# jason-huang03/SPH_Project

Hardware: AMD Instinct MI355X
Metric: particle-updates/sec (higher is better)
Workload: dtype f32

## Files before the change

### include/sph_hip.h

```cpp
#ifndef SPH_HIP_H
#define SPH_HIP_H
#include <stddef.h>
#include <stdint.h>
#ifdef __cplusplus
extern "C" {
#endif

#define SPH_MAX_OBJECTS 20
#define SPH_MAT_FLUID 1
#define SPH_MAT_RIGID 2

typedef enum {
    SPH_OK = 0,
    SPH_ERR_INVALID = -1,
    SPH_ERR_CAPACITY = -2,
    SPH_ERR_HIP = -3,
    SPH_ERR_NO_DEVICE = -4,
    SPH_ERR_COMM = -5,
    SPH_ERR_UNSUPPORTED = -6
} SphStatus;

typedef enum { SPH_METHOD_WCSPH = 0, SPH_METHOD_DFSPH = 1, SPH_METHOD_PCISPH = 2, SPH_METHOD_IISPH = 3, SPH_METHOD_PBF = 4 } SphMethod;

typedef struct {
// ... 81 lines not shown
} SphPhase;

typedef struct {
    int64_t steps;
    int64_t pair_interactions;
    int32_t particle_num;
    int32_t fluid_particle_num;
    int32_t iter_divergence, iter_density, iter_pcisph, iter_cg;
    float   err_divergence, err_density, err_pcisph, err_cg;
    int64_t lds_fallback_blocks;
    double  total_time;
    int64_t pair_evaluations;
    int64_t hash_launches;
    int64_t prehashed_sorts;
    int64_t list_sorts;
    int32_t iter_iisph;
    float   err_iisph;
    int64_t pbf_recentred;
} SphStats;

typedef enum {
    SPH_K_HASH_COUNT = 0, SPH_K_SCAN = 1, SPH_K_SCATTER = 2, SPH_K_DENSITY = 3,
    SPH_K_NON_PRESSURE = 4, SPH_K_PRESSURE_INTEGRATE = 5, SPH_K_RIGID_VOLUME = 6,
    SPH_K_DFSPH_DENSITY_ALPHA = 7, SPH_K_DFSPH_RHO_ADV = 8, SPH_K_DFSPH_CORRECT = 9,
    SPH_K_REDUCE = 10, SPH_K_PCISPH_RHO_STAR = 11, SPH_K_PCISPH_PRESSURE_ACCEL = 12,
    SPH_K_CG_PREPARE = 13, SPH_K_CG_AP = 14, SPH_K_CG_VECTOR = 15, SPH_K_MISC = 16,
    SPH_K_HALO = 17, SPH_K_WCSPH_FORCES = 18,
    SPH_K_IISPH_PREPARE = 19, SPH_K_IISPH_DIJ_PJ = 20, SPH_K_IISPH_SUM_I = 21,
    SPH_K_PBF_DENSITY_LAMBDA = 22, SPH_K_PBF_FIX_POSITION = 23, SPH_K_PBF_UPDATE = 24,
    SPH_K_RIGID_CONTACT = 25, SPH_K_RIGID_INTEGRATE = 26, SPH_K_RIGID_CONTACT_SOLVE = 27, SPH_K_COUNT_
// ... 362 lines not shown
```

### sph_project_amd/_lib.py

```python
from __future__ import annotations

import ctypes as C
import os

import numpy as np

_HERE = os.path.dirname(os.path.abspath(__file__))
LIB_PATH = os.environ.get("SPH_HIP_LIB", os.path.join(_HERE, "libsph_hip.so"))

MAX_OBJECTS = 20
MAT_FLUID, MAT_RIGID = 1, 2
METHOD = {"wcsph": 0, "dfsph": 1, "pcisph": 2, "iisph": 3, "pbf": 4}

(F_POSITION, F_VELOCITY, F_ACCELERATION, F_DENSITY, F_PRESSURE, F_REST_VOLUME, F_MASS, F_MATERIAL,
 F_OBJECT_ID, F_IS_DYNAMIC, F_COLOR, F_PARTICLE_ID, F_GRID_ID, F_DFSPH_ALPHA, F_DFSPH_KAPPA,
 F_DFSPH_KAPPA_V, F_DENSITY_STAR, F_DENSITY_DERIV, F_PRESSURE_ACCEL, F_PREDICTED_VEL, F_PREDICTED_POS,
 F_CG_X, F_ORIG_POSITION, F_GHOST, F_DFSPH_KAPPA_NEXT, F_DFSPH_KAPPA_V_NEXT, F_DEBUG_CAPTURE,
 F_IISPH_DII, F_IISPH_AII, F_IISPH_DIJ_PJ, F_IISPH_SUM_I, F_PBF_OLD_POSITION, F_PBF_LAMBDA, F_RIGID_CONTACT_DN,
 F_RIGID_CONTACT_COUNT) = range(35)

_FIELD_SPEC = {
    F_POSITION: (np.float32, 3), F_VELOCITY: (np.float32, 3), F_ACCELERATION: (np.float32, 3),
    F_DENSITY: (np.float32, 1), F_PRESSURE: (np.float32, 1), F_REST_VOLUME: (np.float32, 1),
    F_MASS: (np.float32, 1), F_MATERIAL: (np.int32, 1), F_OBJECT_ID: (np.int32, 1),
# ... 34 lines not shown
        ("viscosity_b", C.c_double), ("density_0", C.c_double), ("surface_tension", C.c_double),
        ("dt", C.c_double), ("particle_max_num", C.c_int32), ("viscosity_implicit", C.c_int32),
        ("method", C.c_int32), ("fixed_iterations", C.c_int32), ("fast_math", C.c_int32),
        ("device", C.c_int32), ("force_global", C.c_int32), ("deterministic", C.c_int32),
    ]


class SphStats(C.Structure):
    _fields_ = [
        ("steps", C.c_int64), ("pair_interactions", C.c_int64), ("particle_num", C.c_int32),
        ("fluid_particle_num", C.c_int32), ("iter_divergence", C.c_int32), ("iter_density", C.c_int32),
        ("iter_pcisph", C.c_int32), ("iter_cg", C.c_int32), ("err_divergence", C.c_float),
        ("err_density", C.c_float), ("err_pcisph", C.c_float), ("err_cg", C.c_float),
        ("lds_fallback_blocks", C.c_int64), ("total_time", C.c_double), ("pair_evaluations", C.c_int64),
        ("hash_launches", C.c_int64), ("prehashed_sorts", C.c_int64), ("list_sorts", C.c_int64),
        ("iter_iisph", C.c_int32), ("err_iisph", C.c_float), ("pbf_recentred", C.c_int64),
    ]


class SphSurfaceParams(C.Structure):
    _fields_ = [
        ("radius", C.c_double), ("smoothing_length", C.c_double), ("cube_size", C.c_double), ("iso", C.c_double),
        ("normals", C.c_int32), ("fast_math", C.c_int32), ("device", C.c_int32), ("reserved", C.c_int32),
        ("memory_cap_bytes", C.c_int64),
    ]


class SphSurfaceStats(C.Structure):
    _fields_ = [
        ("particles", C.c_int64), ("active_bricks", C.c_int64), ("points_evaluated", C.c_int64), ("pair_tests", C.c_int64),
        ("vertices", C.c_int64), ("triangles", C.c_int64), ("bytes_allocated", C.c_int64), ("B", C.c_int32), ("reserved", C.c_int32),
# ... 555 lines not shown
```

### sph_project_amd/csrc/sph_api.hip

```cpp
#include "../../include/sph_hip.h"
#include "sph_common.hpp"
#include "sph_comm.hpp"

#include <math.h>
#include <stdarg.h>
#include <stdio.h>
#include <string.h>
#include <string>
#include <vector>
#include <stdlib.h>
#include <utility>
#include <array>
#include <algorithm>
#include "sph_voxel.hpp"
#include "sph_export.hpp"
#include "sph_devobj.hpp"

struct ProfSlot {
    bool on = false;
    int64_t launches = 0;
    double ms = 0.0;
    std::vector<std::pair<hipEvent_t, hipEvent_t>> pending;
};

// ... 737 lines not shown
    if (e == hipSuccess) e = hipMemcpyAsync(b, a, bytes, hipMemcpyDeviceToDevice, st);
    if (e == hipSuccess) e = hipEventRecord(e0, st);
    for (int k = 0; k < reps && e == hipSuccess; ++k) e = hipMemcpyAsync((k & 1) ? a : b, (k & 1) ? b : a, bytes, hipMemcpyDeviceToDevice, st);
    if (e == hipSuccess) e = hipEventRecord(e1, st);
    if (e == hipSuccess) e = hipStreamSynchronize(st);
    float ms = 0.0f;
    if (e == hipSuccess) e = hipEventElapsedTime(&ms, e0, e1);
    h->ev_pool.push_back(e0); h->ev_pool.push_back(e1);
    hipFree(a); hipFree(b);
    if (e != hipSuccess || !(ms > 0.0f)) return fail(h, SPH_ERR_HIP, "measure_copy_rate: %s", hipGetErrorString(e));
    *gb_per_s = 2.0 * (double)bytes * reps / ((double)ms * 1e-3) / 1e9;
    return SPH_OK;
}

static int check_async(SphHandle *h) {
    if (h->st.state_error) { const int se = h->st.state_error; h->st.state_error = 0; return fail(h, SPH_ERR_INVALID, "internal state error %d (a sort was scanned without a histogram of its own)", se); }
    hipError_t e = hipGetLastError();
    if (e != hipSuccess) return fail(h, SPH_ERR_HIP, "kernel launch failed: %s", hipGetErrorString(e));
    return SPH_OK;
}

static void ph_neighbor_search(SphHandle *h, bool rho_dead = false) {
    State &s = h->st;
    { ProfScope p(h, SPH_K_HASH_COUNT); h->L->hash_count(s); }
    { ProfScope p(h, SPH_K_SCAN); h->L->scan(s); }
    { ProfScope p(h, SPH_K_SCATTER); if (h->prm.deterministic) h->L->scatter_stable(s, rho_dead); else h->L->scatter(s); }
    h->sort_dirty = false;
}

static void ph_sort_hashed(SphHandle *h) {
    State &s = h->st;
    { ProfScope p(h, SPH_K_SCAN); h->L->scan(s); }
    { ProfScope p(h, SPH_K_SCATTER); if (h->prm.deterministic) h->L->scatter_stable(s, false); else h->L->scatter(s); }
    h->sort_dirty = false;
}

static void ph_rigid_volume(SphHandle *h) {
    if (!h->st.has_rigid) return;
    bool force = false;
    if (h->fresh_state == 2) { h->L->clear_fresh(h->st); h->fresh_state = 0; force = true; }
    else if (h->fresh_state == 1 && h->prm.method != SPH_METHOD_DFSPH) h->fresh_state = 2;
    if (!force && h->rigid_volume_done && !h->st.has_dynamic_rigid) return;
    ProfScope p(h, SPH_K_RIGID_VOLUME);
    h->L->rigid_volume(h->st);
    h->rigid_volume_done = true;
}

static void step_begin(SphHandle *h) {
// ... 235 lines not shown
    return h->n;
}
extern "C" int sph_fluid_particle_num(SphHandle *h) { return h ? h->n_fluid : SPH_ERR_INVALID; }

extern "C" int sph_get_stats(SphHandle *h, SphStats *out) {
    if (!h || !out) return SPH_ERR_INVALID;
    HIPCHK(h, hipSetDevice(h->device));
    int rc = read_scalars(h); if (rc) return rc;
    h->last.steps = h->steps;
    h->last.particle_num = h->n;
    h->last.fluid_particle_num = h->n_fluid;
    h->last.total_time = h->total_time;
    h->last.hash_launches = h->st.n_hash_launches;
    h->last.prehashed_sorts = h->st.n_prehashed_sorts;
    h->last.list_sorts = h->st.n_list_sorts;
    if (h->st.pbf_recentred) {
        unsigned long long r[2];
        HIPCHK(h, hipMemcpy(r, h->st.pbf_recentred, sizeof(r), hipMemcpyDeviceToHost));
        h->last.pbf_recentred = (int64_t)r[h->pbf_bank];
    }
    *out = h->last;
    return SPH_OK;
}

static const float4 *vec_field(SphHandle *h, int field) {
    State &s = h->st;
    switch (field) {
        case SPH_F_POSITION: case SPH_F_REST_VOLUME: return s.posv.cur();
        case SPH_F_VELOCITY: case SPH_F_MASS: return s.velm.cur();
        case SPH_F_ACCELERATION: return s.acc;
// ... 204 lines not shown
```

### sph_project_amd/csrc/sph_common.hpp

```cpp
#pragma once
#include <hip/hip_runtime.h>
#include <stdint.h>

#define SPH_NOBJ 20
#define SPH_IISPH_OMEGA 0.2f
#define SPH_IISPH_ETA 0.001
#define SPH_IISPH_MAX_ITER 20
#define SPH_PBF_LAMBDA_EPS 100.0f
#define SPH_PBF_CORR_K 0.001f
#define SPH_PBF_CORR_DQ 0.3f
#define SPH_PBF_ITERATIONS 5

#define META_OBJ(m) (((m) & 0xff) - 1)
#define META_MAT(m) (((m) >> 8) & 0x3)
#define META_DYN(m) (((m) >> 10) & 0x1)
#define META_PACK(obj, mat, dyn) ((((obj) + 1) & 0xff) | (((mat) & 0x3) << 8) | (((dyn) & 1) << 10))
#define META_GHOST(m) (((m) >> 11) & 0x1)
#define META_DEAD(m) (((m) >> 12) & 0x1)
#define META_FRESH(m) (((m) >> 13) & 0x1)
#define META_FRESH_BIT (1 << 13)
#define META_ACTIVE_FLUID(m) ((((m) >> 8) & 0xB) == 1)
#define META_SET_MAT(m, mat) (((m) & ~(0x3 << 8)) | (((mat) & 0x3) << 8))

struct Consts {
// ... 266 lines not shown
    hipStream_t stream = nullptr;
    int cap = 0;
    DBuf<float4> posv, velm, orig;
    DBuf<int> meta, pid;
    DBuf<unsigned> color;
    DBuf<float> rho;
    int *cell_count = nullptr;
    int *cell_start = nullptr;
    int *cellid = nullptr, *rank = nullptr;
    unsigned long long *run_head = nullptr;
    int2 *run_rec = nullptr;
    unsigned sort_epoch = 0u;
    int run_lists_filed = 0;
    int *sort_inv = nullptr;
    long long n_list_sorts = 0;
    unsigned *color_home = nullptr;
    int color_home_ok = 0, color_stale = 0;
    int *tmp_idx = nullptr;
    int *scan_partial = nullptr;
    int scan_blocks = 0;
    int *scan_tile_state = nullptr;
    int scan_bank = 0;
    int skip_residual = 0;
    int tile_sums_ready = 0;
    int cell_count_clean = 1;
    int hist_taken = 0;
    int state_error = 0;
    float *rho_raw = nullptr, *prs = nullptr, *ptm = nullptr;
    float4 *acc = nullptr;
    float *alpha = nullptr, *kappa = nullptr, *kappa_v = nullptr, *rho_star = nullptr, *rho_deriv = nullptr;
// ... 71 lines not shown
    unsigned char *lane_perm = nullptr;
    int *blk_flag = nullptr, *blk_list = nullptr, *blk_count = nullptr;
    int list_n = -1;
    volatile int *list_count_pinned = nullptr;
    hipEvent_t list_count_event = nullptr;
    int list_count_known = -1;
    int last_pass_listed = 0;
    int *blk_hdr = nullptr;
    int perm_n = -1;
    int has_emitter = 0;
    int visc_rho_raw = 0;
    int skip_viscosity = 0;
    float4 *np_acc_out = nullptr;
};

struct DensityOpts {
    int tiles = 0;
    bool books_forces = false;
};
struct ForceOpts {
    bool booked_by_density = false;
    bool hash_next = false;
};

struct Launch {
    unsigned *(*sorted_color)(State &);
    void (*hash_count)(State &);
    void (*scan)(State &);
    void (*scatter)(State &);
    void (*scatter_stable)(State &, bool rho_dead);
    void (*density)(State &, int eos, DensityOpts o);
    void (*non_pressure)(State &, const float4 *visc_vel);
    void (*pressure_integrate)(State &);
    void (*wcsph_forces)(State &, ForceOpts o);
    void (*rigid_volume)(State &);
    void (*renew_rigid)(State &);
    void (*prepare_emitter)(State &);
    void (*post_insert)(State &, int first, int stale_volume);
    void (*clear_fresh)(State &);
    void (*dfsph_density_alpha)(State &);
    void (*dfsph_density_alpha_div)(State &);
    void (*dfsph_rho_adv)(State &, int mode);
    void (*dfsph_correct)(State &, int mode);
    void (*advect_boundary)(State &, bool hash_next);
    void (*pcisph_init)(State &);
// ... 80 lines not shown
```

### sph_project_amd/csrc/sph_device.hpp

```cpp
#pragma once
#include "sph_common.hpp"
#include <limits.h>

#ifndef SPH_FAST
#define SPH_FAST 0
#endif

__device__ __forceinline__ float fdiv(float a, float b) {
#if SPH_FAST
    return a * __builtin_amdgcn_rcpf(b);
#else
    return a / b;
#endif
}
__device__ __forceinline__ float fdiv2(float a, float b, float c) {
#if SPH_FAST
    return a * __builtin_amdgcn_rcpf(b * c);
#else
    return (a / b) / c;
#endif
}
__device__ __forceinline__ float fsqrt(float a) {
#if SPH_FAST
    return __builtin_amdgcn_sqrtf(a);
// ... 449 lines not shown
template <class P> constexpr bool pass_reuses_masks() { return (PassModes<P>::value & 0b100) != 0; }

template <class P, class = void> struct PassMaskPipe { static constexpr bool value = true; };
template <class P> struct PassMaskPipe<P, decltype((void)P::MASK_PIPELINE)> { static constexpr bool value = P::MASK_PIPELINE; };
template <class P, class = void> struct PassUsesJ0 { static constexpr bool value = true; };
template <class P> struct PassUsesJ0<P, decltype((void)P::USES_J)> { static constexpr bool value = P::USES_J; };
template <class P> constexpr bool pass_mask_pipe() { return PassMaskPipe<P>::value && !(P::HAS_B && PassUsesJ0<P>::value); }
template <class P, class = void> struct PassWrench { static constexpr bool value = false; };
template <class P> struct PassWrench<P, decltype((void)P::HAS_WRENCH)> { static constexpr bool value = P::HAS_WRENCH; };
__device__ __forceinline__ void wrench_init_all(const RigidPose *pose);
__device__ __forceinline__ void wrench_flush_all(DevScalars *scal);
template <class P, class = void> struct PassStatW { static constexpr bool value = false; };
template <class P> struct PassStatW<P, decltype((void)P::STAT_W)> { static constexpr bool value = P::STAT_W; };
template <class P, class = void> struct PassNextHash { static constexpr bool value = false; };
template <class P> struct PassNextHash<P, decltype((void)P::NEXT_HASH)> { static constexpr bool value = P::NEXT_HASH; };
template <class P, class = void> struct PassPrologue { static constexpr bool value = false; };
template <class P> struct PassPrologue<P, decltype((void)P::HAS_PROLOGUE)> { static constexpr bool value = P::HAS_PROLOGUE; };

template <class P, class = void> struct PassC { static constexpr bool value = false; typedef int type; };
template <class P> struct PassC<P, decltype((void)P::HAS_C)> { static constexpr bool value = P::HAS_C; typedef typename P::CT type; };

template <class P>
__device__ __forceinline__ float4 pass_stage(const P &p, const Consts &c, int j, typename P::BT &bj, typename PassC<P>::type &cj) {
    if constexpr (PassC<P>::value) return p.stage(c, j, bj, cj);
    else return p.stage(c, j, bj);
}
template <class P>
__device__ __forceinline__ void pass_pair(const P &p, const Consts &c, typename P::Own &own, float dx, float dy, float dz,
                                          float r2, const float4 &a, const typename P::BT &bj,
                                          const typename PassC<P>::type &cj, int j) {
// ... 290 lines not shown
    }
    block_prep_tile(c, n, p, meta_i, cell_start, blk_hdr, perm, blk_flag, cellw, s_cnt, s_c);
}

__global__ void __launch_bounds__(256)
k_gather_prep(const Consts c, int n, const int *__restrict__ inv, SortArrays a, const int *__restrict__ cell_start,
              int *__restrict__ blk_hdr, unsigned char *__restrict__ perm, int *__restrict__ blk_flag, unsigned *__restrict__ cellw) {
    __shared__ int s_cnt[4][64];
    __shared__ int s_c[2];
    const int d = blockIdx.x * 256 + threadIdx.x;
    float4 p = make_float4(0.f, 0.f, 0.f, 0.f);
    int meta_i = 0;
    if (d < n) {
        const int i = inv[d];
        p = a.posv_in[i];
        meta_i = a.meta_in[i];
        a.posv_out[d] = p;
        a.velm_out[d] = a.velm_in[i];
        a.meta_out[d] = meta_i;
        a.pid_out[d] = a.pid_in[i];
        if (a.color_in) a.color_out[d] = a.color_in[i];
        if (a.rho_in) a.rho_out[d] = a.rho_in[i];
        if (a.orig_in) a.orig_out[d] = a.orig_in[i];
    }
    block_prep_tile(c, n, p, meta_i, cell_start, blk_hdr, perm, blk_flag, cellw, s_cnt, s_c);
}

__global__ void __launch_bounds__(256)
k_color_from_home(int n, const int *__restrict__ pid, const unsigned *__restrict__ home, unsigned *__restrict__ color) {
    const int i = blockIdx.x * 256 + threadIdx.x;
    if (i < n) color[i] = home[pid[i]];
}

__global__ void __launch_bounds__(256)
k_compact_blocks(const int *__restrict__ flag, int nb, int *__restrict__ list, int *__restrict__ count, volatile int *count_host) {
// ... 117 lines not shown
    constexpr int ZW_OFF = (CAP + PAD) * 8;
    __shared__ BT sB[P::HAS_B ? CAP + PAD : 1];
    __shared__ typename PassC<P>::type sC[PassC<P>::value ? CAP + PAD : 1];
    __shared__ unsigned short s_cs[9][NBR_CS_PITCH];
    __shared__ int s_loff[9];

    const int tid = threadIdx.x;
    NBR_STAMP(0);
    const int b = blk_list ? b_listed : xcd_remap(blockIdx.x, nblocks, c.xcd_chunk);
    const int i0 = b * BLOCK;
    const int who_early = lane_perm ? (int)lane_perm[i0 + tid] : tid;
    const int *hdr = blk_hdr + (size_t)b * BLK_HDR_INTS;
    const int cfirst = hdr[0], clast = hdr[1];
    const int skip_tile = tile_skip ? (int)tile_skip[b] : 0;
    const int n_live = live_n(c);
    if constexpr (PassWrench<P>::value) wrench_init_all(p.pose);
    if constexpr (PassPrologue<P>::value) { if (!p.prologue(scal)) return; }
    if (i0 >= n_live) {
        if constexpr (P::HAS_REDUCE) {
            if (tid == 0) {
                const int bs = red_slot(blk_list, b);
                if constexpr (PassSplit<P>::value) {
                    if (gridDim.y > 1) {
                        if (float *o = p.split_out(split_lo((int)gridDim.y, (int)blockIdx.y))) o[bs] = 0.0f;
                        if (gridDim.y == 2 && blockIdx.y == 0) { if (float *o = p.split_out(1)) o[bs] = 0.0f; }
                    } else p.red_out[bs] = 0.0f;
                }
                else p.red_out[bs] = 0.0f;
            }
        }
        return;
    }
    const int who = who_early;
    const int i = i0 + who;
    const bool valid = i < n_live;

    const int span = clast - cfirst;
    bool cs_lds = span >= 0 && span <= NBR_CS_SPAN;
#pragma unroll
    for (int k = 0; k < 9; ++k) cs_lds = cs_lds && hdr[11 + k] < 65536;
    const int ic = valid ? i : i0;
    const unsigned cw = reinterpret_cast<const unsigned *>(blk_hdr + (size_t)((mask_stride + 255) >> 8) * BLK_HDR_INTS)[ic];
    const float4 pi = p.posv[ic];
    Own own;
    bool active = p.begin(c, ic, pi, own) && valid;
    unsigned mk0[3] = {0u, 0u, 0u};
    if (MASKMODE == 2 && pass_mask_pipe<P>()) {
        const int g0 = (PassSplit<P>::value && gridDim.y > 1) ? split_lo((int)gridDim.y, (int)blockIdx.y) : 0;
#pragma unroll
        for (int q = 0; q < 3; ++q) mk0[q] = nbr_mask[(size_t)run_of(c.run_grouping, g0, q) * mask_stride + i];
    }
    typedef typename PassC<P>::type CT;
    const int g_first = (PassSplit<P>::value && gridDim.y > 1) ? split_lo((int)gridDim.y, (int)blockIdx.y) : 0;
    (void)g_first;
    if (cs_lds && tid < NBR_CS_PITCH) {
        const int tc = tid < span + 4 ? tid : span + 3;
        int cs_[9];
#pragma unroll
        for (int k = 0; k < 9; ++k) {
            int cell = cfirst + (k / 3 - 1) * c.ny * c.nz + (k % 3 - 1) * c.nz - 1 + tc;
            cell = cell < 0 ? 0 : (cell > c.G ? c.G : cell);
            cs_[k] = cell_start[cell];
        }
        if (tid < span + 4) {
#pragma unroll
            for (int k = 0; k < 9; ++k) s_cs[k][tid] = (unsigned short)(cs_[k] - hdr[2 + k]);
        }
    }
    const int e0 = (int)(cw & 0xffu);
    const int e1 = e0 + (int)((cw >> 8) & 7u);
    const unsigned dom = cw >> 11;
    if (skip_tile) return;
    if (__syncthreads_or(active ? 1 : 0)) {
        NBR_STAMP(1);
        unsigned npairs = 0;
        const bool is_split = PassSplit<P>::value && gridDim.y > 1;
        const int g_lo = is_split ? split_lo((int)gridDim.y, (int)blockIdx.y) : 0;
        const int g_hi = is_split ? split_hi((int)gridDim.y, (int)blockIdx.y) : GROUPS;
        unsigned mkn[RPG] = {mk0[0], mk0[1], mk0[2]};
#pragma unroll 1
        for (int g = g_lo, qa = 0; g < (c.force_global == 11 ? 0 : g_hi); ) {
            int rs_[RPG], ln_[RPG], lo_[RPG];
            int total, qb;
            unsigned rm;
            bool overflow;
            nbr_plan<CAP>(hdr, g, qa, c.force_global, rs_, ln_, lo_, total, qb, rm, overflow, c.run_grouping);
#define NBR_IN_ROUND(q) ((rm >> (q)) & 1u)
            if (tid < RPG) {
// ... 278 lines not shown
```

### sph_project_amd/csrc/sph_kernels.hip

```cpp
#include "sph_common.hpp"

#if SPH_FAST
#define SPH_LAUNCH_FN sph_launch_fast
#define SPH_NS sph_fast_ns
#else
#define SPH_LAUNCH_FN sph_launch_strict
#define SPH_NS sph_strict_ns
#endif

#include <vector>
#include <cstdio>
#include <cstdint>
namespace SPH_NS {
#include "sph_device.hpp"
#include "sph_halo_defs.hpp"
#include "sph_passes.hpp"
#include "sph_solvers.hpp"
#include "sph_cg.hpp"
#include "sph_halo.hpp"

inline int cdiv(int a, int b) { return (a + b - 1) / b; }

static int *tile_sum_bank(State &s) {
    if (s.slab_active) return nullptr;
// ... 77 lines not shown
        s.list_count_known = -1;
        if (s.list_count_event) hipEventRecord(s.list_count_event, s.stream);
    }
    s.list_n = lst ? n : -1;
    s.perm_n = n;
}

unsigned *l_sorted_color(State &s) {
    if (s.color_stale) {
        s.color_stale = 0;
        if (s.c.n > 0) hipLaunchKernelGGL(k_color_from_home, dim3(cdiv(s.c.n, 256)), dim3(256), 0, s.stream, s.c.n, s.pid.cur(), s.color_home, s.color.cur());
    }
    return s.color.cur();
}

void l_scatter_impl(State &s, bool stable, bool rho_dead) {
    const int n = s.c.n;
    if (n == 0) return;
    SortArrays a;
    a.G = s.c.G;
    a.posv_in = s.posv.cur(); a.posv_out = s.posv.alt();
    a.velm_in = s.velm.cur(); a.velm_out = s.velm.alt();
    a.meta_in = s.meta.cur(); a.meta_out = s.meta.alt();
    a.pid_in = s.pid.cur(); a.pid_out = s.pid.alt();
    a.color_out = s.color.alt();
    a.rho_in = s.rho.cur(); a.rho_out = s.rho.alt();
    a.orig_in = s.orig.cur(); a.orig_out = s.orig.alt();
    a.xidx_in = s.slab_active ? s.xidx[s.xcur] : nullptr; a.xidx_out = s.slab_active ? s.xidx[1 - s.xcur] : nullptr;
    const bool by_lists = stable && s.run_lists_filed && s.run_head && s.sort_inv && !s.slab_active;
    a.color_in = by_lists ? s.color.cur() : l_sorted_color(s);
    s.run_lists_filed = 0;
    const bool skip_rho = by_lists && rho_dead && s.c.all_fluid;
    if (by_lists) {
        if (s.color_home && s.color_home_ok) { a.color_in = nullptr; s.color_stale = 1; }
        if (skip_rho) a.rho_in = nullptr;
        hipLaunchKernelGGL(k_sort_rank, dim3(cdiv(n, 256)), dim3(256), 0, s.stream, n, s.cellid, s.cell_start,
                           RunList{s.run_head, s.run_rec, s.cap, s.sort_epoch}, s.sort_inv);
        const bool lst = !s.c.all_fluid && s.blk_list;
        hipLaunchKernelGGL(k_gather_prep, dim3(cdiv(n, 256)), dim3(256), 0, s.stream, s.c, n, s.sort_inv, a, s.cell_start,
                           s.blk_hdr, s.lane_perm, lst ? s.blk_flag : nullptr,
                           reinterpret_cast<unsigned *>(s.blk_hdr + (size_t)((s.cap + 255) / 256) * BLK_HDR_INTS));
        s.n_list_sorts++;
    } else if (stable) {
        hipLaunchKernelGGL(k_scatter_index, dim3(cdiv(n, 256)), dim3(256), 0, s.stream, n, s.cellid, s.rank,
                           s.cell_start, (int2 *)s.tmp_idx, s.c.n_dev);
        hipLaunchKernelGGL(k_scatter<true>, dim3(cdiv(n, 256)), dim3(256), 0, s.stream, n, s.cellid, s.rank,
                           s.cell_start, (const int2 *)s.tmp_idx, a, s.c.n_dev);
    } else {
        hipLaunchKernelGGL(k_scatter<false>, dim3(cdiv(n, 256)), dim3(256), 0, s.stream, n, s.cellid, s.rank,
                           s.cell_start, (const int2 *)s.tmp_idx, a, s.c.n_dev);
    }
    s.posv.flip(); s.velm.flip(); s.meta.flip(); s.pid.flip(); s.color.flip(); s.rho.flip();
#ifdef SPH_TEST_HOOKS
    if (skip_rho) hipMemsetAsync(s.rho.cur(), 0xFF, sizeof(float) * (size_t)n, s.stream);
#endif
    s.masks_valid = 0;
    if (!s.slab_active) l_block_prep(s, !by_lists);
    else s.perm_n = s.list_n = -1;
    if (s.orig.cur()) s.orig.flip();
    if (s.slab_active) s.xcur = 1 - s.xcur;
}
void l_scatter(State &s) { l_scatter_impl(s, false, false); }
void l_scatter_stable(State &s, bool rho_dead) { l_scatter_impl(s, true, rho_dead); }

int list_grid(State &s, int nb) {
    if (!s.list_count_pinned) return nb;
    if (s.list_count_known < 0 && s.list_count_event) {
        const hipError_t q = hipEventQuery(s.list_count_event);
        if (q == hipSuccess) s.list_count_known = *s.list_count_pinned;
        else if (q == hipErrorNotReady && hipPeekAtLastError() == hipErrorNotReady) (void)hipGetLastError();
    }
    const int g = s.list_count_known >= 0 ? s.list_count_known : nb;
    return g < 1 ? 1 : (g > nb ? nb : g);
}

template <class P> void launch_pass(State &s, const P &p, int mask_mode = 0, int tiles = 0, int split = 0) {
    const int n = s.c.n;
    if (n == 0) return;
// ... 43 lines not shown
                if (t[15] > tmax) tmax = t[15];
            }
            double life = 0; for (int b = 0; b < nb; ++b) life += (double)(hbuf[(size_t)b * 16 + 15] - hbuf[(size_t)b * 16]);
            fprintf(stderr, "timeline mode %d BT %d: kernel %.1f kclk, workgroup lifetime %.1f kclk; mean clk per stamp:", mask_mode, (int)sizeof(typename P::BT), (tmax - tmin) * 1e-3, life / nb * 1e-3);
            for (int k = 1; k < 16; ++k) fprintf(stderr, " [%d]%.0f", k, cnt[k] ? d[k] / cnt[k] : 0.0);
            fprintf(stderr, "\n");
        }
    }
}

void l_density(State &s, int eos, DensityOpts o) {
    HaloFieldSend fs = s.fieldsend;
    if (!eos) fs.on = 0;
    s.fieldsend.on = 0;
    const int sp = o.books_forces ? 1 + 3 : 1, se = o.books_forces ? 2 : 1;
    if (s.c.all_fluid) {
        if (eos) { DensityPass<true, true> p{s.posv.cur(), s.meta.cur(), s.rho_raw, s.rho.cur(), s.prs, s.ptm, fs, sp, se}; launch_pass(s, p, 1, o.tiles); }
        else { DensityPass<true, false> p{s.posv.cur(), s.meta.cur(), s.rho_raw, s.rho.cur(), s.prs, s.ptm, fs, sp, se}; launch_pass(s, p, 1, o.tiles); }
    } else {
        if (eos) { DensityPass<false, true> p{s.posv.cur(), s.meta.cur(), s.rho_raw, s.rho.cur(), s.prs, s.ptm, fs, sp, se}; launch_pass(s, p, 1, o.tiles); }
        else { DensityPass<false, false> p{s.posv.cur(), s.meta.cur(), s.rho_raw, s.rho.cur(), s.prs, s.ptm, fs, sp, se}; launch_pass(s, p, 1, o.tiles); }
    }
}

void l_non_pressure(State &s, const float4 *visc_vel) {
    const float *rho_src = s.visc_rho_raw ? s.rho_raw : s.rho.cur();
    if (s.poly6) {
        if (s.c.all_fluid) {
            NonPressurePass<true, Poly6Kernel> p{s.posv.cur(), s.velm.cur(), s.meta.cur(), rho_src, s.velm.alt(), s.scal, s.pose, s.c.rho0, s.skip_viscosity, s.np_acc_out, visc_vel};
            launch_pass(s, p, 2);
        } else {
            NonPressurePass<false, Poly6Kernel> p{s.posv.cur(), s.velm.cur(), s.meta.cur(), rho_src, s.velm.alt(), s.scal, s.pose, s.c.rho0, s.skip_viscosity, s.np_acc_out, visc_vel};
            launch_pass(s, p, 2);
        }
    } else if (s.c.all_fluid) {
        NonPressurePass<true> p{s.posv.cur(), s.velm.cur(), s.meta.cur(), rho_src, s.velm.alt(), s.scal, s.pose, s.c.rho0, s.skip_viscosity, s.np_acc_out, visc_vel};
// ... 216 lines not shown
```

### sph_project_amd/csrc/sph_passes.hpp

```cpp
#pragma once
#include "sph_device.hpp"

typedef float WrenchRows[4][SPH_NOBJ][6];
__device__ __forceinline__ WrenchRows &wrench_rows() {
    __shared__ WrenchRows s_rows;
    return s_rows;
}
typedef float WrenchCom[SPH_NOBJ][3];
__device__ __forceinline__ WrenchCom &wrench_com() {
    __shared__ WrenchCom s_com;
    return s_com;
}
__device__ __forceinline__ void wrench_init_all(const RigidPose *pose) {
    float *r = &wrench_rows()[0][0][0];
    for (int k = threadIdx.x; k < 4 * SPH_NOBJ * 6; k += 256) r[k] = 0.0f;
    if (threadIdx.x < SPH_NOBJ * 3) (&wrench_com()[0][0])[threadIdx.x] = (&pose->com[0][0])[threadIdx.x];
}
__device__ __forceinline__ void wrench_flush_all(DevScalars *scal) {
    const int k = threadIdx.x;
    if (k >= SPH_NOBJ * 6) return;
    const WrenchRows &w = wrench_rows();
    const int obj = k / 6, q = k % 6;
    const float v = ((w[0][obj][q] + w[1][obj][q]) + w[2][obj][q]) + w[3][obj][q];
    if (v != 0.0f)
        atomicAdd((unsigned long long *)(scal->wrench + (q < 3 ? 0 : SPH_NOBJ * 3) + obj * 3 + q % 3),
                  (unsigned long long)__double2ll_rn((double)v * SPH_WRENCH_SCALE));
}
__device__ __forceinline__ void add_wrench(DevScalars *, int obj, float fx, float fy, float fz, float tx, float ty, float tz) {
    float *r = wrench_rows()[threadIdx.x >> 6][obj];
    atomicAdd(r + 0, fx); atomicAdd(r + 1, fy); atomicAdd(r + 2, fz);
    atomicAdd(r + 3, tx); atomicAdd(r + 4, ty); atomicAdd(r + 5, tz);
}

template <bool AF, bool EOS>
struct DensityPass {
    static constexpr int MODES = 0b011;
    static constexpr bool FLUID_BLOCKS_ONLY = true;
    static constexpr int BLOCK = 256, GROUPS = 3;
    static constexpr bool USES_J = !AF;
    static constexpr bool HAS_B = false, COUNT_PAIRS = true;
    static constexpr int PAIR_WEIGHT = 1;
    static constexpr bool HAS_REDUCE = false;
    typedef int BT;
    struct Own { float sum; };
    const float4 *posv; const int *meta;
    float *rho_raw, *rho, *prs, *ptm;
    HaloFieldSend fs;
    static constexpr bool STAT_W = true;
    int stat_pairs, stat_evals;

    __device__ float4 loadA(int j) const { return posv[j]; }
    __device__ BT loadB(int) const { return 0; }
    __device__ float4 stage(const Consts &, int j, BT &) const { return posv[j]; }
    __device__ bool begin(const Consts &c, int i, const float4 &, Own &o) const {
        o.sum = 0.0f;
        if (AF && !c.ghosts) return true;
        return META_ACTIVE_FLUID(meta[i]);
    }
    __device__ void pair(const Consts &c, Own &o, float, float, float, float r2, const float4 &a, const BT &,
                         int) const {
#if SPH_FAST
        const float q2 = r2 * c.inv_h2, q = __builtin_amdgcn_sqrtf(q2), t = 1.0f - q;
        const float lo = 1.0f - (6.0f * q2) * t, hi = 2.0f * (t * t * t);
        o.sum += a.w * (q <= 0.5f ? lo : hi);
// ... 555 lines not shown
```

### sph_project_amd/csrc/sph_steps.hpp

```cpp
#pragma once
#include <sched.h>

static int read_red(SphHandle *h, int slot, float *out) {
    HIPCHK(h, hipMemcpyAsync(&h->scal_h->red[slot], &h->st.scal->red[slot], sizeof(float), hipMemcpyDeviceToHost, h->st.stream));
    HIPCHK(h, hipStreamSynchronize(h->st.stream));
    *out = h->scal_h->red[slot];
    return SPH_OK;
}

static int implicit_viscosity_non_pressure(SphHandle *h);

struct LoopPub { float red[8]; int flags[4]; unsigned seq; unsigned pad[3]; };
static_assert(sizeof(LoopPub) == 64, "LoopPub layout");
__global__ void __launch_bounds__(64) k_publish_loop(DevScalars *scal, LoopPub *pub, unsigned seq) {
    const int t = threadIdx.x;
    const int stop = scal->flags[0];
    if (t < 8) __hip_atomic_store(&pub->red[t], scal->red[t], __ATOMIC_RELAXED, __HIP_MEMORY_SCOPE_SYSTEM);
    else if (t < 12) __hip_atomic_store(&pub->flags[t - 8], scal->flags[t - 8], __ATOMIC_RELAXED, __HIP_MEMORY_SCOPE_SYSTEM);
    __threadfence_system();
    __syncthreads();
    if (t == 0) {
        if (stop) { scal->flags[0] = 0; scal->flags[1] = 0; }
        __hip_atomic_store(&pub->seq, seq, __ATOMIC_RELEASE, __HIP_MEMORY_SCOPE_SYSTEM);
    }
// ... 112 lines not shown
}

static int run_non_pressure(SphHandle *h) {
    if (h->prm.viscosity_implicit) {
        int rc = implicit_viscosity_non_pressure(h);
        return rc;
    }
    ProfScope p(h, SPH_K_NON_PRESSURE);
    h->L->non_pressure(h->st, nullptr);
    return SPH_OK;
}

static int wcsph_step(SphHandle *h) {
    State &s = h->st;
    const bool fused = !h->prm.viscosity_implicit;
    if (s.slab_active) { int rc = slab_neighbor_search(h, fused); if (rc) return rc; }
    else ph_neighbor_search(h, true);
    ph_rigid_volume(h);
    const bool books = fused && !getenv("SPH_FORCES_COUNT_OWN");
    const bool overlap = s.slab_active && s.push.on && s.tile_list[0] && s.c.all_fluid && s.tile_plan_n == s.c.n && (s.has_down || s.has_up);
    if (overlap) {
        const int hint = slab_field_hint(h);
        { ProfScope p(h, SPH_K_DENSITY); h->L->density(s, 1, {1, books}); }
        { ProfScope p(h, SPH_K_HALO); h->L->halo_push_fields(s, 2, nullptr, nullptr, hint); }
        { ProfScope p(h, SPH_K_DENSITY); h->L->density(s, 1, {2, books}); }
        { ProfScope p(h, SPH_K_HALO); h->L->halo_pull_fields(s, 2, nullptr, nullptr, hint); }
    } else if (s.slab_active && s.push.on) {
        const int hint = slab_field_hint(h);
        h->L->halo_fieldsend_begin(s);
        { ProfScope p(h, SPH_K_DENSITY); h->L->density(s, 1, {0, books}); }
        { ProfScope p(h, SPH_K_HALO); h->L->halo_pull_fields(s, 2, nullptr, nullptr, hint); }
    } else {
        { ProfScope p(h, SPH_K_DENSITY); h->L->density(s, 1, {0, books}); }
        if (s.slab_active) { int rc = slab_exchange_fields(h); if (rc) return rc; }
    }
    if (fused) {
        const SlabComm &cm = h->comm;
        const bool rebalance_next = cm.rebalance_every > 0 && (h->steps + 1) % cm.rebalance_every == 0 && !h->any_rigid_object;
        if (s.slab_active && s.push.on && h->steps_to_follow > 0 && !rebalance_next && !s.has_emitter && !h->any_rigid_object &&
            !h->sort_dirty)
            h->L->halo_presend_begin(s);
        const bool hash_next = !s.slab_active && s.c.all_fluid && h->steps_to_follow > 0 && !s.has_emitter && !h->any_rigid_object &&
                               !h->sort_dirty;
        ProfScope p(h, SPH_K_WCSPH_FORCES); h->L->wcsph_forces(s, {books, hash_next});
        return SPH_OK;
    }
    int rc = run_non_pressure(h); if (rc) return rc;
    { ProfScope p(h, SPH_K_PRESSURE_INTEGRATE); h->L->pressure_integrate(s); }
// ... 72 lines not shown
    const SolveSpec sp{.slot = 2, .kind = 2, .thr = 0.001,
                       .denom = (float)(s.slab_active ? h->comm_nfluid_global : (long long)h->n_fluid),
                       .max_itr = 1000, .fixed_err = 100.0f,
                       .iter = &h->last.iter_pcisph, .err = &h->last.err_pcisph, .batch_end = nullptr};
    return run_solve(h, sp, [] {}, [&]() -> int {
        { ProfScope p(h, SPH_K_PCISPH_RHO_STAR); h->L->pcisph_rho_star(s); }
        if (s.slab_active) { int rc = slab_exchange_scalar(h, s.ptm); if (rc) return rc; }
        { ProfScope p(h, SPH_K_PCISPH_PRESSURE_ACCEL); h->L->pcisph_pressure_accel(s); }
        if (s.slab_active) { int rc = slab_exchange_vel(h, s.ppos); if (rc) return rc; }
        return s.slab_active ? slab_finish_reduction(h, 2) : SPH_OK;
    });
}

static int pcisph_step(SphHandle *h) {
    State &s = h->st;
    if (s.slab_active) { int rc = slab_neighbor_search(h); if (rc) return rc; }
    else ph_neighbor_search(h, true);
    ph_rigid_volume(h);
    { ProfScope p(h, SPH_K_DENSITY); h->L->density(s, 0, {}); }
    if (s.slab_active) { int rc = slab_exchange_scalar(h, s.rho.cur()); if (rc) return rc; }
    int rc = run_non_pressure(h); if (rc) return rc;
    { ProfScope p(h, SPH_K_MISC); h->L->pcisph_init(s); }
    if (s.slab_active) { rc = slab_exchange_vel(h, s.ppos); if (rc) return rc; }
    rc = pcisph_refine(h); if (rc) return rc;
    { ProfScope p(h, SPH_K_PRESSURE_INTEGRATE); h->L->pressure_integrate(s); }
    return SPH_OK;
}

static void iisph_iteration(SphHandle *h) {
    State &s = h->st;
    { ProfScope p(h, SPH_K_IISPH_DIJ_PJ); h->L->iisph_dij_pj(s); }
    { ProfScope p(h, SPH_K_IISPH_SUM_I); h->L->iisph_sum_i(s); }
}

static int iisph_refine(SphHandle *h) {
    const SolveSpec sp{.slot = 2, .kind = 2, .thr = SPH_IISPH_ETA, .denom = (float)h->n_fluid * (float)h->prm.density_0,
                       .max_itr = SPH_IISPH_MAX_ITER, .fixed_err = 0.0f, .iter = &h->last.iter_iisph, .err = &h->last.err_iisph,
                       .batch_end = nullptr};
    return run_solve(h, sp, [] {}, [h] { iisph_iteration(h); return (int)SPH_OK; });
}

static int iisph_step(SphHandle *h) {
    State &s = h->st;
    ph_neighbor_search(h, true);
    ph_rigid_volume(h);
    { ProfScope p(h, SPH_K_DENSITY); h->L->density(s, 0, {}); }
    int rc = run_non_pressure(h); if (rc) return rc;
    { ProfScope p(h, SPH_K_IISPH_PREPARE); h->L->iisph_prepare(s); }
    rc = iisph_refine(h); if (rc) return rc;
    { ProfScope p(h, SPH_K_PRESSURE_INTEGRATE); h->L->pressure_integrate(s); }
    return SPH_OK;
}

static void pbf_begin_count(SphHandle *h) {
    State &s = h->st;
    h->pbf_bank = s.c.stat_bank;
    hipMemsetAsync(s.pbf_recentred + s.c.stat_bank, 0, sizeof(unsigned long long), s.stream);
}

static int pbf_step(SphHandle *h) {
    State &s = h->st;
// ... 91 lines not shown
```

Baseline: 5.162 billion.

## Defer velocity/meta/pid permutation from sort scatter into density kernel

When sorting by lists in deterministic mode and a density pass follows, the scatter kernel now skips gathering velocity, meta and particle-id arrays. The density kernel performs that gather itself, one element per thread, so the extra memory traffic overlaps with the neighbor loop. The goal is to cut scatter bandwidth and hide the gather latency inside density. It adds register pressure in density, is limited to all-fluid runs without tile lists, and sets an error flag when a carry cannot be honored.

After: 5.257 billion, median of 6. 1.02x the previous value.

```diff
diff --git a/include/sph_hip.h b/include/sph_hip.h
--- a/include/sph_hip.h
+++ b/include/sph_hip.h
@@ -119,6 +119,7 @@
     int64_t hash_launches;
     int64_t prehashed_sorts;
     int64_t list_sorts;
+    int64_t carried_sorts;
     int32_t iter_iisph;
     float   err_iisph;
     int64_t pbf_recentred;
diff --git a/sph_project_amd/_lib.py b/sph_project_amd/_lib.py
--- a/sph_project_amd/_lib.py
+++ b/sph_project_amd/_lib.py
@@ -72,7 +72,7 @@
         ("err_density", C.c_float), ("err_pcisph", C.c_float), ("err_cg", C.c_float),
         ("lds_fallback_blocks", C.c_int64), ("total_time", C.c_double), ("pair_evaluations", C.c_int64),
         ("hash_launches", C.c_int64), ("prehashed_sorts", C.c_int64), ("list_sorts", C.c_int64),
-        ("iter_iisph", C.c_int32), ("err_iisph", C.c_float), ("pbf_recentred", C.c_int64),
+        ("carried_sorts", C.c_int64), ("iter_iisph", C.c_int32), ("err_iisph", C.c_float), ("pbf_recentred", C.c_int64),
     ]
 
 
diff --git a/sph_project_amd/csrc/sph_api.hip b/sph_project_amd/csrc/sph_api.hip
--- a/sph_project_amd/csrc/sph_api.hip
+++ b/sph_project_amd/csrc/sph_api.hip
@@ -775,24 +775,26 @@
 }
 
 static int check_async(SphHandle *h) {
-    if (h->st.state_error) { const int se = h->st.state_error; h->st.state_error = 0; return fail(h, SPH_ERR_INVALID, "internal state error %d (a sort was scanned without a histogram of its own)", se); }
+    if (h->st.state_error) { const int se = h->st.state_error; h->st.state_error = 0; return fail(h, SPH_ERR_INVALID, "internal state error %d (bit 0: a sort was scanned without a histogram of its own; bit 1: a density launch could not move the arrays its sort left to it)", se); }
     hipError_t e = hipGetLastError();
     if (e != hipSuccess) return fail(h, SPH_ERR_HIP, "kernel launch failed: %s", hipGetErrorString(e));
     return SPH_OK;
 }
 
-static void ph_neighbor_search(SphHandle *h, bool rho_dead = false) {
-    State &s = h->st;
+static SortCarry ph_neighbor_search(SphHandle *h, bool rho_dead = false, bool density_next = false) {
+    State &s = h->st;
+    SortCarry carry;
     { ProfScope p(h, SPH_K_HASH_COUNT); h->L->hash_count(s); }
     { ProfScope p(h, SPH_K_SCAN); h->L->scan(s); }
-    { ProfScope p(h, SPH_K_SCATTER); if (h->prm.deterministic) h->L->scatter_stable(s, rho_dead); else h->L->scatter(s); }
+    { ProfScope p(h, SPH_K_SCATTER); if (h->prm.deterministic) carry = h->L->scatter_stable(s, rho_dead, density_next && !getenv("SPH_NO_SORT_CARRY")); else h->L->scatter(s); }
     h->sort_dirty = false;
+    return carry;
 }
 
 static void ph_sort_hashed(SphHandle *h) {
     State &s = h->st;
     { ProfScope p(h, SPH_K_SCAN); h->L->scan(s); }
-    { ProfScope p(h, SPH_K_SCATTER); if (h->prm.deterministic) h->L->scatter_stable(s, false); else h->L->scatter(s); }
+    { ProfScope p(h, SPH_K_SCATTER); if (h->prm.deterministic) h->L->scatter_stable(s, false, false); else h->L->scatter(s); }
     h->sort_dirty = false;
 }
 
@@ -1058,6 +1060,7 @@
     h->last.hash_launches = h->st.n_hash_launches;
     h->last.prehashed_sorts = h->st.n_prehashed_sorts;
     h->last.list_sorts = h->st.n_list_sorts;
+    h->last.carried_sorts = h->st.n_carried_sorts;
     if (h->st.pbf_recentred) {
         unsigned long long r[2];
         HIPCHK(h, hipMemcpy(r, h->st.pbf_recentred, sizeof(r), hipMemcpyDeviceToHost));
diff --git a/sph_project_amd/csrc/sph_common.hpp b/sph_project_amd/csrc/sph_common.hpp
--- a/sph_project_amd/csrc/sph_common.hpp
+++ b/sph_project_amd/csrc/sph_common.hpp
@@ -304,6 +304,7 @@
     int run_lists_filed = 0;
     int *sort_inv = nullptr;
     long long n_list_sorts = 0;
+    long long n_carried_sorts = 0;
     unsigned *color_home = nullptr;
     int color_home_ok = 0, color_stale = 0;
     int *tmp_idx = nullptr;
@@ -405,9 +406,20 @@
     float4 *np_acc_out = nullptr;
 };
 
+struct SortCarry {
+    const int *inv = nullptr;
+    const float4 *velm_in = nullptr; float4 *velm_out = nullptr;
+    const int *meta_in = nullptr; int *meta_out = nullptr;
+    const int *pid_in = nullptr; int *pid_out = nullptr;
+    int on = 0;
+};
+template <bool ON> struct SortCarryOf { SortCarry carry; };
+template <> struct SortCarryOf<false> {};
+
 struct DensityOpts {
     int tiles = 0;
     bool books_forces = false;
+    SortCarry carry = {};
 };
 struct ForceOpts {
     bool booked_by_density = false;
@@ -419,7 +431,7 @@
     void (*hash_count)(State &);
     void (*scan)(State &);
     void (*scatter)(State &);
-    void (*scatter_stable)(State &, bool rho_dead);
+    SortCarry (*scatter_stable)(State &, bool rho_dead, bool density_next);
     void (*density)(State &, int eos, DensityOpts o);
     void (*non_pressure)(State &, const float4 *visc_vel);
     void (*pressure_integrate)(State &);
diff --git a/sph_project_amd/csrc/sph_device.hpp b/sph_project_amd/csrc/sph_device.hpp
--- a/sph_project_amd/csrc/sph_device.hpp
+++ b/sph_project_amd/csrc/sph_device.hpp
@@ -487,6 +487,8 @@
 template <class P> struct PassStatW<P, decltype((void)P::STAT_W)> { static constexpr bool value = P::STAT_W; };
 template <class P, class = void> struct PassNextHash { static constexpr bool value = false; };
 template <class P> struct PassNextHash<P, decltype((void)P::NEXT_HASH)> { static constexpr bool value = P::NEXT_HASH; };
+template <class P, class = void> struct PassSortCarry { static constexpr bool value = false; };
+template <class P> struct PassSortCarry<P, decltype((void)P::SORT_CARRY)> { static constexpr bool value = P::SORT_CARRY; };
 template <class P, class = void> struct PassPrologue { static constexpr bool value = false; };
 template <class P> struct PassPrologue<P, decltype((void)P::HAS_PROLOGUE)> { static constexpr bool value = P::HAS_PROLOGUE; };
 
@@ -807,11 +809,13 @@
     if (d < n) {
         const int i = inv[d];
         p = a.posv_in[i];
-        meta_i = a.meta_in[i];
         a.posv_out[d] = p;
-        a.velm_out[d] = a.velm_in[i];
-        a.meta_out[d] = meta_i;
-        a.pid_out[d] = a.pid_in[i];
+        if (a.velm_in) {
+            meta_i = a.meta_in[i];
+            a.velm_out[d] = a.velm_in[i];
+            a.meta_out[d] = meta_i;
+            a.pid_out[d] = a.pid_in[i];
+        }
         if (a.color_in) a.color_out[d] = a.color_in[i];
         if (a.rho_in) a.rho_out[d] = a.rho_in[i];
         if (a.orig_in) a.orig_out[d] = a.orig_in[i];
@@ -959,6 +963,14 @@
     const int cfirst = hdr[0], clast = hdr[1];
     const int skip_tile = tile_skip ? (int)tile_skip[b] : 0;
     const int n_live = live_n(c);
+    int carry_d = 0;
+    unsigned carry_src = 0u;
+    if constexpr (PassSortCarry<P>::value) {
+        if (p.carry.on) {
+            carry_d = i0 + tid;
+            carry_src = (unsigned)p.carry.inv[carry_d < c.n ? carry_d : c.n - 1];
+        }
+    }
     if constexpr (PassWrench<P>::value) wrench_init_all(p.pose);
     if constexpr (PassPrologue<P>::value) { if (!p.prologue(scal)) return; }
     if (i0 >= n_live) {
@@ -989,6 +1001,11 @@
     const float4 pi = p.posv[ic];
     Own own;
     bool active = p.begin(c, ic, pi, own) && valid;
+    float4 carry_v = make_float4(0.f, 0.f, 0.f, 0.f);
+    int carry_m = 0, carry_p = 0;
+    if constexpr (PassSortCarry<P>::value) {
+        if (p.carry.on) { carry_v = p.carry.velm_in[carry_src]; carry_m = p.carry.meta_in[carry_src]; carry_p = p.carry.pid_in[carry_src]; }
+    }
     unsigned mk0[3] = {0u, 0u, 0u};
     if (MASKMODE == 2 && pass_mask_pipe<P>()) {
         const int g0 = (PassSplit<P>::value && gridDim.y > 1) ? split_lo((int)gridDim.y, (int)blockIdx.y) : 0;
@@ -1016,7 +1033,14 @@
     const int e1 = e0 + (int)((cw >> 8) & 7u);
     const unsigned dom = cw >> 11;
     if (skip_tile) return;
-    if (__syncthreads_or(active ? 1 : 0)) {
+    if constexpr (PassSortCarry<P>::value) {
+        asm volatile("" :: "v"(cw), "v"(pi.w), "v"(carry_v.x), "v"(carry_m), "v"(carry_p));
+    }
+    const int any_active = __syncthreads_or(active ? 1 : 0);
+    if constexpr (PassSortCarry<P>::value) {
+        if (p.carry.on && carry_d < c.n) { p.carry.velm_out[carry_d] = carry_v; p.carry.meta_out[carry_d] = carry_m; p.carry.pid_out[carry_d] = carry_p; }
+    }
+    if (any_active) {
         NBR_STAMP(1);
         unsigned npairs = 0;
         const bool is_split = PassSplit<P>::value && gridDim.y > 1;
diff --git a/sph_project_amd/csrc/sph_kernels.hip b/sph_project_amd/csrc/sph_kernels.hip
--- a/sph_project_amd/csrc/sph_kernels.hip
+++ b/sph_project_amd/csrc/sph_kernels.hip
@@ -115,9 +115,10 @@
     return s.color.cur();
 }
 
-void l_scatter_impl(State &s, bool stable, bool rho_dead) {
+SortCarry l_scatter_impl(State &s, bool stable, bool rho_dead, bool density_next) {
     const int n = s.c.n;
-    if (n == 0) return;
+    SortCarry carry;
+    if (n == 0) return carry;
     SortArrays a;
     a.G = s.c.G;
     a.posv_in = s.posv.cur(); a.posv_out = s.posv.alt();
@@ -132,9 +133,17 @@
     a.color_in = by_lists ? s.color.cur() : l_sorted_color(s);
     s.run_lists_filed = 0;
     const bool skip_rho = by_lists && rho_dead && s.c.all_fluid;
+    carry.on = by_lists && density_next && s.c.all_fluid && !s.tile_list[0];
     if (by_lists) {
         if (s.color_home && s.color_home_ok) { a.color_in = nullptr; s.color_stale = 1; }
         if (skip_rho) a.rho_in = nullptr;
+        if (carry.on) {
+            carry.inv = s.sort_inv;
+            carry.velm_in = a.velm_in; carry.velm_out = a.velm_out;
+            carry.meta_in = a.meta_in; carry.meta_out = a.meta_out;
+            carry.pid_in = a.pid_in; carry.pid_out = a.pid_out;
+            a.velm_in = nullptr; a.meta_in = nullptr; a.pid_in = nullptr;
+        }
         hipLaunchKernelGGL(k_sort_rank, dim3(cdiv(n, 256)), dim3(256), 0, s.stream, n, s.cellid, s.cell_start,
                            RunList{s.run_head, s.run_rec, s.cap, s.sort_epoch}, s.sort_inv);
         const bool lst = !s.c.all_fluid && s.blk_list;
@@ -154,15 +163,21 @@
     s.posv.flip(); s.velm.flip(); s.meta.flip(); s.pid.flip(); s.color.flip(); s.rho.flip();
 #ifdef SPH_TEST_HOOKS
     if (skip_rho) hipMemsetAsync(s.rho.cur(), 0xFF, sizeof(float) * (size_t)n, s.stream);
+    if (carry.on) {
+        hipMemsetAsync(s.velm.cur(), 0xFF, sizeof(float4) * (size_t)n, s.stream);
+        hipMemsetAsync(s.meta.cur(), 0xFF, sizeof(int) * (size_t)n, s.stream);
+        hipMemsetAsync(s.pid.cur(), 0xFF, sizeof(int) * (size_t)n, s.stream);
+    }
 #endif
     s.masks_valid = 0;
     if (!s.slab_active) l_block_prep(s, !by_lists);
     else s.perm_n = s.list_n = -1;
     if (s.orig.cur()) s.orig.flip();
     if (s.slab_active) s.xcur = 1 - s.xcur;
-}
-void l_scatter(State &s) { l_scatter_impl(s, false, false); }
-void l_scatter_stable(State &s, bool rho_dead) { l_scatter_impl(s, true, rho_dead); }
+    return carry;
+}
+void l_scatter(State &s) { l_scatter_impl(s, false, false, false); }
+SortCarry l_scatter_stable(State &s, bool rho_dead, bool density_next) { return l_scatter_impl(s, true, rho_dead, density_next); }
 
 int list_grid(State &s, int nb) {
     if (!s.list_count_pinned) return nb;
@@ -236,12 +251,18 @@
     if (!eos) fs.on = 0;
     s.fieldsend.on = 0;
     const int sp = o.books_forces ? 1 + 3 : 1, se = o.books_forces ? 2 : 1;
+    SortCarry carry = o.carry;
+    if (carry.on && (!s.c.all_fluid || o.tiles != 0 || s.c.n == 0)) { s.state_error |= 2; carry.on = 0; }
+#ifdef SPH_TEST_HOOKS
+    if (getenv("SPH_TEST_DROP_CARRY")) carry.on = 0;
+#endif
+    if (carry.on) s.n_carried_sorts++;
     if (s.c.all_fluid) {
-        if (eos) { DensityPass<true, true> p{s.posv.cur(), s.meta.cur(), s.rho_raw, s.rho.cur(), s.prs, s.ptm, fs, sp, se}; launch_pass(s, p, 1, o.tiles); }
-        else { DensityPass<true, false> p{s.posv.cur(), s.meta.cur(), s.rho_raw, s.rho.cur(), s.prs, s.ptm, fs, sp, se}; launch_pass(s, p, 1, o.tiles); }
-    } else {
-        if (eos) { DensityPass<false, true> p{s.posv.cur(), s.meta.cur(), s.rho_raw, s.rho.cur(), s.prs, s.ptm, fs, sp, se}; launch_pass(s, p, 1, o.tiles); }
-        else { DensityPass<false, false> p{s.posv.cur(), s.meta.cur(), s.rho_raw, s.rho.cur(), s.prs, s.ptm, fs, sp, se}; launch_pass(s, p, 1, o.tiles); }
+        if (eos) { DensityPass<true, true> p{{carry}, s.posv.cur(), s.meta.cur(), s.rho_raw, s.rho.cur(), s.prs, s.ptm, fs, sp, se}; launch_pass(s, p, 1, o.tiles); }
+        else { DensityPass<true, false> p{{carry}, s.posv.cur(), s.meta.cur(), s.rho_raw, s.rho.cur(), s.prs, s.ptm, fs, sp, se}; launch_pass(s, p, 1, o.tiles); }
+    } else {
+        if (eos) { DensityPass<false, true> p{{}, s.posv.cur(), s.meta.cur(), s.rho_raw, s.rho.cur(), s.prs, s.ptm, fs, sp, se}; launch_pass(s, p, 1, o.tiles); }
+        else { DensityPass<false, false> p{{}, s.posv.cur(), s.meta.cur(), s.rho_raw, s.rho.cur(), s.prs, s.ptm, fs, sp, se}; launch_pass(s, p, 1, o.tiles); }
     }
 }
 
diff --git a/sph_project_amd/csrc/sph_passes.hpp b/sph_project_amd/csrc/sph_passes.hpp
--- a/sph_project_amd/csrc/sph_passes.hpp
+++ b/sph_project_amd/csrc/sph_passes.hpp
@@ -33,7 +33,7 @@
 }
 
 template <bool AF, bool EOS>
-struct DensityPass {
+struct DensityPass : SortCarryOf<AF> {
     static constexpr int MODES = 0b011;
     static constexpr bool FLUID_BLOCKS_ONLY = true;
     static constexpr int BLOCK = 256, GROUPS = 3;
@@ -48,6 +48,7 @@
     HaloFieldSend fs;
     static constexpr bool STAT_W = true;
     int stat_pairs, stat_evals;
+    static constexpr bool SORT_CARRY = AF;
 
     __device__ float4 loadA(int j) const { return posv[j]; }
     __device__ BT loadB(int) const { return 0; }
diff --git a/sph_project_amd/csrc/sph_steps.hpp b/sph_project_amd/csrc/sph_steps.hpp
--- a/sph_project_amd/csrc/sph_steps.hpp
+++ b/sph_project_amd/csrc/sph_steps.hpp
@@ -150,8 +150,9 @@
 static int wcsph_step(SphHandle *h) {
     State &s = h->st;
     const bool fused = !h->prm.viscosity_implicit;
+    SortCarry carry;
     if (s.slab_active) { int rc = slab_neighbor_search(h, fused); if (rc) return rc; }
-    else ph_neighbor_search(h, true);
+    else carry = ph_neighbor_search(h, true, true);
     ph_rigid_volume(h);
     const bool books = fused && !getenv("SPH_FORCES_COUNT_OWN");
     const bool overlap = s.slab_active && s.push.on && s.tile_list[0] && s.c.all_fluid && s.tile_plan_n == s.c.n && (s.has_down || s.has_up);
@@ -167,7 +168,7 @@
         { ProfScope p(h, SPH_K_DENSITY); h->L->density(s, 1, {0, books}); }
         { ProfScope p(h, SPH_K_HALO); h->L->halo_pull_fields(s, 2, nullptr, nullptr, hint); }
     } else {
-        { ProfScope p(h, SPH_K_DENSITY); h->L->density(s, 1, {0, books}); }
+        { ProfScope p(h, SPH_K_DENSITY); h->L->density(s, 1, {0, books, carry}); }
         if (s.slab_active) { int rc = slab_exchange_fields(h); if (rc) return rc; }
     }
     if (fused) {
@@ -270,10 +271,11 @@
 
 static int pcisph_step(SphHandle *h) {
     State &s = h->st;
+    SortCarry carry;
     if (s.slab_active) { int rc = slab_neighbor_search(h); if (rc) return rc; }
-    else ph_neighbor_search(h, true);
+    else carry = ph_neighbor_search(h, true, true);
     ph_rigid_volume(h);
-    { ProfScope p(h, SPH_K_DENSITY); h->L->density(s, 0, {}); }
+    { ProfScope p(h, SPH_K_DENSITY); h->L->density(s, 0, {0, false, carry}); }
     if (s.slab_active) { int rc = slab_exchange_scalar(h, s.rho.cur()); if (rc) return rc; }
     int rc = run_non_pressure(h); if (rc) return rc;
     { ProfScope p(h, SPH_K_MISC); h->L->pcisph_init(s); }
@@ -298,9 +300,9 @@
 
 static int iisph_step(SphHandle *h) {
     State &s = h->st;
-    ph_neighbor_search(h, true);
+    const SortCarry carry = ph_neighbor_search(h, true, true);
     ph_rigid_volume(h);
-    { ProfScope p(h, SPH_K_DENSITY); h->L->density(s, 0, {}); }
+    { ProfScope p(h, SPH_K_DENSITY); h->L->density(s, 0, {0, false, carry}); }
     int rc = run_non_pressure(h); if (rc) return rc;
     { ProfScope p(h, SPH_K_IISPH_PREPARE); h->L->iisph_prepare(s); }
     rc = iisph_refine(h); if (rc) return rc;
```
